# StephenNG59/ICP-symm

Measured on AMD Instinct MI355X. Metric: icp_iterations_per_sec, higher is better.
Workload: dtype f32

## Files before the change

icp-symm_amd/csrc/engine.cpp:

```cpp
#include "engine_internal.h"
#include "robust_loss.h"
#include <limits>

void read_switches(Switches &w)
{
    auto flag = [](const char *n) { return std::getenv(n) != nullptr; };
    auto num = [](const char *n, long def) { const char *e = std::getenv(n); return e ? std::atol(e) : def; };
    auto tri = [](const char *n) { const char *e = std::getenv(n); return e ? (e[0] == '1' ? 1 : 0) : -1; };
    w.allow_any_arch = flag("SYMMICP_ALLOW_ANY_ARCH");
    w.debug_host = flag("SYMMICP_DEBUG_HOST");
    w.debug_counters = flag("SYMMICP_DEBUG_COUNTERS");
    if (const char *e = std::getenv("SYMMICP_DEBUG_TRACE")) w.debug_trace = e;
    if (const char *e = std::getenv("SYMMICP_GRID_PPC")) w.grid_ppc = std::atof(e);
    w.grid_maxlevel = (int)num("SYMMICP_GRID_MAXLEVEL", kMortonBits);
    w.grid_level = (int)num("SYMMICP_GRID_LEVEL", -1);
    if (const char *e = std::getenv("SYMMICP_FIRST_PASS")) w.first_pass = (e[0] == 'p') ? 1 : 0;
    w.oct_leaf = (int)num("SYMMICP_OCT_LEAF", 0);
    if (const char *e = std::getenv("SYMMICP_PACKET_ORDER")) w.packet_order = e[0] != '0';
    if (const char *e = std::getenv("SYMMICP_PACKET_JUMP")) w.packet_jump = (float)std::atof(e);
    w.packet_key_bits = (int)num("SYMMICP_PACKET_KEY_BITS", 16);
    w.packet_chunk = (uint32_t)num("SYMMICP_PACKET_CHUNK", 0);
    w.packet_lds_pad = (uint32_t)num("SYMMICP_PACKET_LDS_PAD", 0);
    w.packet_waves = (uint32_t)num("SYMMICP_PACKET_WAVES", 0);
    w.packet_front_cap = (uint32_t)num("SYMMICP_PACKET_FRONT_CAP", 0);
    if (const char *e = std::getenv("SYMMICP_HOOD_FRAC")) w.hood_frac = std::atof(e);
    w.no_hood = flag("SYMMICP_NO_NEIGHBOURHOOD");
    w.no_cert = flag("SYMMICP_NO_CERT");
    w.walk_full_grid = flag("SYMMICP_WALK_FULL_GRID");
    { const char *e = std::getenv("SYMMICP_HOST_LOOP"); w.host_loop = e && e[0] == '1'; }
    w.no_loop_stragglers = flag("SYMMICP_NO_LOOP_STRAGGLERS");
    w.force_comm = flag("SYMMICP_FORCE_COMM");
    if (const char *e = std::getenv("SYMMICP_PACKET_COST_KEY")) w.packet_cost_key = e[0] != '0';
    w.budget_walk = tri("SYMMICP_BUDGET_WALK");
    w.optimistic = tri("SYMMICP_OPTIMISTIC");
    w.compact = tri("SYMMICP_COMPACT");
    w.pass_blocks = (int)num("SYMMICP_PASS_BLOCKS", 2048);
    w.id_blocks = (int)num("SYMMICP_ID_BLOCKS", 2048);
    w.acc_blocks = (int)num("SYMMICP_ACC_BLOCKS", 512);
    w.fused_blocks = (int)num("SYMMICP_FUSED_BLOCKS", 512);
    w.compact_blocks = (int)num("SYMMICP_COMPACT_BLOCKS", 1280);
    w.feature_nn_splits = (int)num("SYMMICP_FEATURE_NN_SPLITS", 0);
    w.feature_nn_queries = (int)num("SYMMICP_FEATURE_NN_QUERIES", 0);
    w.tune.wave_mode_max = (uint32_t)num("SYMMICP_WAVE_MODE_MAX", 20000);
    w.tune.cells_chunk = (uint32_t)num("SYMMICP_CELLS_CHUNK", 16);
    w.tune.cells_queries = (uint32_t)num("SYMMICP_CELLS_QUERIES", 0);
    w.tune.walk_budget = (uint32_t)num("SYMMICP_WALK_BUDGET", 160);
}

void arena_begin(Arena &a, size_t want)
{
    a.off = 0;
    if (a.cap >= want) return;
    if (a.base) hipFree(a.base);
    a.base = nullptr; a.cap = 0;
    const size_t cap = want + want / 4;
    if (hipMalloc((void **)&a.base, cap) == hipSuccess) a.cap = cap;
    else (void)hipGetLastError();
}


extern "C" {

int symmicp_version(void) { return 100; }

void symmicp_config_default(symmicp_config *cfg)
{
    if (!cfg) return;
    std::memset(cfg, 0, sizeof(*cfg));
    cfg->struct_size = (int32_t)sizeof(*cfg);
    cfg->device = -1;
    cfg->mode = SYMMICP_MODE_QUIRKS;
    cfg->corr = SYMMICP_CORR_IDENTITY;
    cfg->apply = SYMMICP_APPLY_DEFAULT;
    cfg->max_iters = 10;
    cfg->diff_threshold = 1.0f;
    cfg->max_corr_dist = 0.f;
    cfg->fixed_iters = 0;
// ... 1387 lines not shown
```

icp-symm_amd/csrc/engine_debug.cpp:

```cpp
#include "engine_internal.h"

static constexpr size_t kTraceWords = (size_t)1 << 22;
void dump_packet_trace(symmicp_ctx *c)
{
    if (FILE *f = std::fopen(c->sw.debug_trace.c_str(), "wb")) {
        std::vector<unsigned long long> t(kTraceWords);
        hipMemcpy(t.data(), c->dbg_trace, t.size() * 8, hipMemcpyDeviceToHost);
        std::fwrite(t.data(), 8, t.size(), f);
        std::fclose(f);
    }
    hipMemset(c->dbg_trace, 0, kTraceWords * 8);
}


void print_pass_counters(symmicp_ctx *c, bool first, long long list_len)
{
        unsigned long long h[12];
        hipMemcpy(h, c->ix.dbg, sizeof(h), hipMemcpyDeviceToHost);
        hipMemset(c->ix.dbg, 0, sizeof(h));
        if (first && c->cfg.corr == SYMMICP_CORR_TREE && c->target_surface_like)
            std::fprintf(stderr, "[symmicp dbg] pass %lld (packets): steps=%llu nodes+leaf candidates=%llu leaf candidates rejected=%llu points=%llu tie rescans=%llu overflows=%llu lanes wanting a scanned leaf (sum)=%llu | packet ticks (10 ns): sum=%llu max=%llu\n",
                         (long long)c->st.passes, h[0], h[4], h[5], h[3], h[2], h[1], h[8], h[7], h[6]);
        else
        std::fprintf(stderr, "[symmicp dbg] pass %lld: cells: certified=%llu (by neighbourhood %llu) scans=%llu (neighbourhoods kept %llu, not kept %llu) probes=%llu to-walk=%llu items=%llu points=%llu | walk list=%lld visits=%llu wave-max*64=%llu\n",
                     (long long)c->st.passes, h[1], h[8], h[2], h[9], h[10], h[6], h[7], h[0], h[3], list_len, h[4], h[5]);
}
```

icp-symm_amd/csrc/engine_internal.h:

```cpp
#pragma once
#include <hip/hip_runtime.h>
#include <dlfcn.h>
#include <fcntl.h>
#include <sys/mman.h>
#include <sys/stat.h>
#include <unistd.h>
#include <algorithm>
#include <chrono>
#include <cmath>
#include <cstdio>
#include <cstdlib>
#include <cstring>
#include <mutex>
#include <string>
#include <vector>

#include "symmicp.h"
#include "symmicp_internal.h"
#include "host_solve.h"


namespace symmicp {}
using namespace symmicp;

// ... 2 lines not shown
typedef int (*fn_ncclGetUniqueId)(rcclUniqueId *);
typedef int (*fn_ncclCommInitRank)(rcclComm_t *, int, rcclUniqueId, int);
typedef int (*fn_ncclCommDestroy)(rcclComm_t);
typedef int (*fn_ncclAllReduce)(const void *, void *, size_t, int, int, rcclComm_t, hipStream_t);
typedef const char *(*fn_ncclGetErrorString)(int);
constexpr int kNcclFloat64 = 8;
constexpr int kNcclSum = 0;

struct Rccl {
    void *handle = nullptr;
    fn_ncclGetUniqueId GetUniqueId = nullptr;
    fn_ncclCommInitRank CommInitRank = nullptr;
    fn_ncclCommDestroy CommDestroy = nullptr;
    fn_ncclAllReduce AllReduce = nullptr;
    fn_ncclGetErrorString GetErrorString = nullptr;
    std::string err;
    std::mutex mu;
    bool load()
    {
        std::lock_guard<std::mutex> lock(mu);
        if (handle && AllReduce) return true;
        const char *names[] = {"librccl.so.1", "librccl.so"};
        for (const char *nm : names) { handle = dlopen(nm, RTLD_NOW | RTLD_NOLOAD | RTLD_GLOBAL); if (handle) break; }
        if (!handle)
            for (const char *nm : names) { handle = dlopen(nm, RTLD_NOW | RTLD_GLOBAL); if (handle) break; }
        if (!handle) { err = std::string("cannot load librccl: ") + dlerror(); return false; }
        GetUniqueId = (fn_ncclGetUniqueId)dlsym(handle, "ncclGetUniqueId");
        CommInitRank = (fn_ncclCommInitRank)dlsym(handle, "ncclCommInitRank");
        CommDestroy = (fn_ncclCommDestroy)dlsym(handle, "ncclCommDestroy");
        AllReduce = (fn_ncclAllReduce)dlsym(handle, "ncclAllReduce");
        GetErrorString = (fn_ncclGetErrorString)dlsym(handle, "ncclGetErrorString");
        if (!GetUniqueId || !CommInitRank || !CommDestroy || !AllReduce) { err = "librccl misses nccl* symbols"; return false; }
        return true;
    }
};
extern Rccl g_rccl;

inline double now_s()
{
    return std::chrono::duration<double>(std::chrono::steady_clock::now().time_since_epoch()).count();
}

struct Switches {
    bool allow_any_arch = false, debug_host = false, debug_counters = false;
    std::string debug_trace;
    double grid_ppc = 3.0;
    int grid_maxlevel = kMortonBits, grid_level = -1;
    int first_pass = -1;
    int oct_leaf = 0;
    bool packet_order = true;
    bool packet_cost_key = true;
    float packet_jump = -1.0f;
    int packet_key_bits = 16;
    uint32_t packet_chunk = 0, packet_lds_pad = 0, packet_waves = 0, packet_front_cap = 0;
    double hood_frac = 0.8;
    bool no_hood = false, no_cert = false, walk_full_grid = false, host_loop = false, no_loop_stragglers = false, force_comm = false;
    int budget_walk = -1, optimistic = -1, compact = -1;
    int pass_blocks = 2048, id_blocks = 2048, acc_blocks = 512, fused_blocks = 512, compact_blocks = 1280;
    int feature_nn_splits = 0, feature_nn_queries = 0;
    PassTuning tune;
};

void read_switches(Switches &w);

struct Arena {
    char *base = nullptr;
    size_t cap = 0, off = 0;
};

struct ShmSlot {
    volatile unsigned long long seq;
    double s[SYMMICP_NSUM];
    char pad[512 - 8 - 8 * SYMMICP_NSUM];
};
static_assert(sizeof(ShmSlot) == 512, "slot = 4 cache lines");
struct ShmExchange {
    ShmSlot *slots = nullptr;
    size_t bytes = 0;
    unsigned long long count = 0;
    std::string name;
    bool owner = false;
};

struct IndexNotes {
    float origin[3] = {0, 0, 0}, h0 = 0.f;
    uint32_t hist[16] = {};
    uint32_t leaf_max = 0;
    uint32_t nblocks = 0, ctop_len = 0;
};

struct symmicp_ctx {
    Switches sw;
    Arena arena;
    Arena keep;
    std::vector<void *> keep_extra;
    ShmExchange shm;
    symmicp_config cfg{};
    int loss = SYMMICP_LOSS_NONE;
    float loss_scale = 0.f;
    float gicp_eps = 1e-3f;
    float color_lam = 0.968f;
    float4 *tgt_color = nullptr;
    float *src_int = nullptr;
    size_t tgt_color_cap = 0, src_int_cap = 0;
    bool have_tgt_color = false, have_src_int = false;
    float trim_frac = 1.0f;
    uint32_t *trim_keys = nullptr, *trim_ws = nullptr;
// ... 139 lines not shown
```

icp-symm_amd/csrc/engine_loop.cpp:

```cpp
#include "engine_internal.h"

extern "C" {

static void fill_pass_args(symmicp_ctx *c, PassArgs &a, const float Xapply[16], bool from_cur, bool writeback, bool first)
{
    a.in = from_cur ? c->cur : c->src0;
    a.out = c->cur;
    a.n = c->n_loc;
    a.tgt_offset = c->src_off;
    for (int k = 0; k < 12; k++) a.X.m[k] = Xapply[k];
    a.X.nrm_w = (c->cfg.mode == SYMMICP_MODE_QUIRKS) ? 1.0f : 0.0f;
    const bool paper = c->cfg.mode != SYMMICP_MODE_QUIRKS;
    for (int k = 0; k < 3; k++) a.pivot[k] = paper ? c->pivot[k] : 0.0f;
    a.p2p = c->cfg.mode == SYMMICP_MODE_P2P ? 1 : 0;
    a.obj = mode_obj(c->cfg.mode);
    a.gicp_k = 1.0f - c->gicp_eps;
    a.tgt_color = c->tgt_color;
    a.src_int = c->src_int;
    a.color_lam = c->color_lam;
    a.color_om = 1.0f - c->color_lam;
    a.max_d2 = c->cfg.max_corr_dist > 0.f ? c->cfg.max_corr_dist * c->cfg.max_corr_dist : 0.f;
    a.min_ndot = c->cfg.min_normal_dot;
    a.writeback = writeback ? 1 : 0;
    a.best64 = c->best64;
    a.pos_prev = first ? nullptr : c->pos;
    a.pos_out = c->pos;
    a.d2_out = (c->cfg.corr == SYMMICP_CORR_IDENTITY) ? nullptr : c->d2;
    a.partials = c->partials;
    a.cert = reinterpret_cast<float4 *>(c->cert);
    a.certk = c->sw.no_hood ? nullptr : reinterpret_cast<uint4 *>(c->certk);
    a.hoodr = reinterpret_cast<float2 *>(c->hoodr);
    a.make_hood = (a.certk && !first && c->last_uncertified >= 0 && (double)c->last_uncertified < c->sw.hood_frac * (double)c->n_s_total) ? 1 : 0;
    a.pairrec = c->pairrec;
    a.budget_walk = c->sw.budget_walk >= 0 ? c->sw.budget_walk : (first && c->nranks > 1 && c->n_loc < 400000u);
    a.use_slack = (!first && c->cert && !c->sw.no_cert) ? 1 : 0;
    a.loop = nullptr;
    a.pkt_tab = reinterpret_cast<const uint2 *>(c->pkt_tab);
    a.pkt_count = c->pkt_count;
    a.pkt_waves = c->sw.packet_waves;
    a.pkt_front_cap = c->sw.packet_front_cap;
    a.pkt_fallbacks = c->pkt_fallbacks;
    a.pkt_chunk = c->sw.packet_chunk;
    a.pkt_lds_pad = c->sw.packet_lds_pad;
    a.loss = c->loss;
    a.loss_scale = c->loss_scale;
    const bool trim = c->trim_frac < 1.0f && c->trim_keys && c->trim_ws;
    a.trim_keys = trim ? c->trim_keys : nullptr;
    a.trim_ws = trim ? c->trim_ws : nullptr;
    a.trim_host = trim ? reinterpret_cast<uint32_t *>(c->h_sums_dev + kNSum + 1) : nullptr;
    a.trim_rho = c->trim_frac;
}

static int run_pass(symmicp_ctx *c, const float Xapply[16], bool from_cur, bool writeback, bool first)
{
    const bool trim = c->trim_frac < 1.0f;
    if (trim) {
        const size_t want = c->n_loc ? c->n_loc : 1;
        if (c->trim_keys_cap < want) {
            hipFree(c->trim_keys);
            c->trim_keys = nullptr; c->trim_keys_cap = 0;
            HIP_TRY(c, hipMalloc((void **)&c->trim_keys, sizeof(uint32_t) * want));
            c->trim_keys_cap = want;
        }
        if (!c->trim_ws) HIP_TRY(c, hipMalloc((void **)&c->trim_ws, sizeof(uint32_t) * kTrimWsWords));
    }
    c->trim_valid = false;
    PassArgs a{};
    fill_pass_args(c, a, Xapply, from_cur, writeback, first);
    int blocks = (int)((c->n_loc + kPassThreads - 1) / kPassThreads);
    int cap = c->sw.pass_blocks;
    if (cap > 8192) cap = 8192;
    if (blocks > cap) blocks = cap;
    if (blocks < 1) blocks = 1;
    c->pass_blocks = blocks;
    const double t_l0 = now_s();
    if (c->t_last_done > 0) c->t_between += t_l0 - c->t_last_done;
    hipEvent_t *ev = nullptr;
    uint32_t walk_blocks = 0;
    bool optimistic = false;
    if (c->timing) {
        if (c->ev_used == symmicp_ctx::kEvRing) flush_events(c);
        ev = c->ev + c->ev_used * symmicp_ctx::kEvPer;
        c->ev_split[c->ev_used] = (c->timing == 1 || c->timing == 3) ? 1 : 0;
        c->ev_weight[c->ev_used] = 1;
    }
    if (ev && !(c->timing == 2 && c->cfg.corr == SYMMICP_CORR_TREE)) hipEventRecord(ev[0], c->stream);
    switch (c->cfg.corr) {
    case SYMMICP_CORR_IDENTITY: {
        const bool vec4 = (c->n_loc % 4 == 0) && (c->n_t % 4 == 0) && (c->src_off % 4 == 0);
        if (vec4) {
            const int id_cap = c->sw.id_blocks;
            const int nb4 = (int)((c->n_loc / 4 + kPassThreads - 1) / kPassThreads);
            blocks = nb4 < id_cap ? (nb4 > 0 ? nb4 : 1) : id_cap;
// ... 617 lines not shown
```

icp-symm_amd/csrc/kernels_packet.hip:

```cpp
#include <cstdlib>
#include "symmicp_internal.h"
#include "device_common.h"
#pragma clang fp contract(off)

namespace symmicp {

constexpr int kPktStack = 128;
static_assert(kPktStack >= 7 * (kMortonBits + 1) + 1, "packet stack too small for the octree depth");

typedef float f32x16 __attribute__((ext_vector_type(16)));

__device__ __forceinline__ void sload_2x16(const void *p, f32x16 &a, f32x16 &b)
{
    const unsigned long long u = (unsigned long long)p;
    p = (const void *)(((unsigned long long)(uint32_t)__builtin_amdgcn_readfirstlane((int)(u >> 32)) << 32) |
                       (unsigned long long)(uint32_t)__builtin_amdgcn_readfirstlane((int)(uint32_t)u));
    asm volatile("s_load_dwordx16 %0, %2, 0x0\n\ts_load_dwordx16 %1, %2, 0x40\n\ts_waitcnt lgkmcnt(0)" : "=&s"(a), "=&s"(b) : "s"(p) : "memory");
}

template <int CTRL, int ROW_MASK>
__device__ __forceinline__ uint32_t dpp_umax(uint32_t x)
{
    return max(x, (uint32_t)__builtin_amdgcn_update_dpp(0, (int)x, CTRL, ROW_MASK, 0xf, false));
}
// ... 46 lines not shown
{
    const float d2 = dist2(px, py, pz, qx, qy, qz);
    const bool lt = d2 < b.d2;
    tie |= __ballot(d2 == b.d2);
    if (CERT) b.second = min(b.second, max(__float_as_uint(d2), __float_as_uint(b.d2)));
    b.d2 = lt ? d2 : b.d2;
    slot = lt ? K : slot;
}


template <bool CERT>
__device__ __forceinline__ void pkt_leaf_scalar(const float4 *__restrict__ tq, uint32_t first, uint32_t cnt, float px, float py, float pz,
                                                PktBest &b, unsigned long long &c_tie)
{
    for (uint32_t e0 = 0; e0 < cnt; e0 += 8) {
        const uint32_t m = min(cnt - e0, 8u);
        f32x16 qa, qb;
        sload_2x16(tq + first + e0, qa, qb);
        int32_t slot = 8;
        unsigned long long tie = 0;
        pkt_point<CERT, 0>(b, slot, tie, px, py, pz, qa[0], qa[1], qa[2]);
        if (m > 1u) pkt_point<CERT, 1>(b, slot, tie, px, py, pz, qa[4], qa[5], qa[6]);
        if (m > 2u) pkt_point<CERT, 2>(b, slot, tie, px, py, pz, qa[8], qa[9], qa[10]);
        if (m > 3u) pkt_point<CERT, 3>(b, slot, tie, px, py, pz, qa[12], qa[13], qa[14]);
        if (m > 4u) pkt_point<CERT, 4>(b, slot, tie, px, py, pz, qb[0], qb[1], qb[2]);
        if (m > 5u) pkt_point<CERT, 5>(b, slot, tie, px, py, pz, qb[4], qb[5], qb[6]);
        if (m > 6u) pkt_point<CERT, 6>(b, slot, tie, px, py, pz, qb[8], qb[9], qb[10]);
        if (m > 7u) pkt_point<CERT, 7>(b, slot, tie, px, py, pz, qb[12], qb[13], qb[14]);
        if (slot != 8) b.pos = (int32_t)(first + e0) + slot;
        if (tie != 0ull) {
            c_tie++;
            int32_t brow = (b.pos >= 0) ? __float_as_int(tq[b.pos].w) : 0x7fffffff;
#pragma unroll
            for (int k = 0; k < 8; k++) {
                if ((uint32_t)k < m) {
                    const float qx = k < 4 ? qa[4 * k] : qb[4 * (k - 4)], qy = k < 4 ? qa[4 * k + 1] : qb[4 * (k - 4) + 1],
                                qz = k < 4 ? qa[4 * k + 2] : qb[4 * (k - 4) + 2];
                    const int32_t row = __float_as_int(k < 4 ? qa[4 * k + 3] : qb[4 * (k - 4) + 3]);
                    const float d2 = dist2(px, py, pz, qx, qy, qz);
                    if (d2 == b.d2 && row < brow) { brow = row; b.pos = (int32_t)(first + e0) + k; }
                }
            }
        }
    }
}

__device__ __forceinline__ float bcast(float v, int src_lane)
{
    return __int_as_float(__builtin_amdgcn_readlane(__float_as_int(v), src_lane));
}

struct PktCounters {
    unsigned long long nodes, leaves, rejected, points, ties, steps, overflow, wantlanes;
};

template <bool CERT>
__device__ __noinline__ void pkt_dfs(const float4 *__restrict__ onodes, const float4 *__restrict__ tq, const uint32_t *s_off, float4 (*stk)[2],
                                     const float (*s_sb)[8], uint8_t *s_lvl, const int lane, float px, float py, float pz, PktBest &b, float &thr, float pad, PktCounters &cn)
{
    const int sub = lane & 3, chl = lane >> 2;
    const int bperm = (16 * sub + 15) * 4;
    const float4 sblo = *reinterpret_cast<const float4 *>(&s_sb[sub][0]), sbhi = *reinterpret_cast<const float4 *>(&s_sb[sub][4]);
    if (lane == 0) {
        const float4 rA = onodes[0], rB = onodes[1];
        stk[0][0] = rA; stk[0][1] = rB;
        s_lvl[0] = 0;
    }
    int sp = 1;
    __builtin_amdgcn_wave_barrier();
    while (sp > 0) {
        sp--;
        const float4 nA = stk[sp][0], nB = stk[sp][1];
        const bool want = boxdist2(px, py, pz, nA, nB) <= thr;
        if (__ballot(want) == 0ull) { cn.rejected++; continue; }
        const uint32_t first = (uint32_t)__builtin_amdgcn_readfirstlane(__float_as_int(nA.w));
        const uint32_t packed = (uint32_t)__builtin_amdgcn_readfirstlane(__float_as_int(nB.w));
        const uint32_t level = s_lvl[sp], nch = oct_nch(packed), cf = oct_cf(packed);
        if (nch == 0) {
            cn.leaves++; cn.points += cf;
            pkt_leaf_scalar<CERT>(tq, first, cf, px, py, pz, b, cn.ties);
            thr = fminf(thr, pkt_threshold(b.d2, pad));
        } else {
            cn.nodes++;
            const uint32_t tb = (thr >= 0.0f) ? __float_as_uint(thr) + 1u : 0u;
            const uint32_t thr_g = (uint32_t)__builtin_amdgcn_ds_bpermute(bperm, (int)row_umax(tb));
            uint32_t bbd = 0x7f800000u;
            float4 cA = make_float4(0.f, 0.f, 0.f, 0.f), cB = cA;
            const bool mine = (lane < 32) && ((uint32_t)chl < nch);
            if (mine) {
                const float4 *__restrict__ ch = onodes + 2 * ((size_t)s_off[level + 1] + cf + (uint32_t)chl);
                cA = ch[0]; cB = ch[1];
                const float gx = fmaxf(fmaxf(cA.x - sbhi.x, sblo.x - cB.x), 0.0f);
                const float gy = fmaxf(fmaxf(cA.y - sbhi.y, sblo.y - cB.y), 0.0f);
                const float gz = fmaxf(fmaxf(cA.z - sbhi.z, sblo.z - cB.z), 0.0f);
                bbd = __float_as_uint((gx * gx + gy * gy) + gz * gz);
            }
            const bool keep = mine && bbd < thr_g;
            const uint32_t m32 = (uint32_t)__ballot(keep);
            if (m32) {
                uint32_t mc = m32 | (m32 >> 1);
                mc = (mc | (mc >> 2)) & 0x11111111u;
                uint32_t key = keep ? ((bbd & ~7u) | (uint32_t)chl) : 0xFFFFFFFFu;
                key = dpp_umin<0xB1, 0xf>(key);
                key = dpp_umin<0x4E, 0xf>(key);
                key = dpp_umin<0x114, 0xf>(key);
                key = dpp_umin<0x118, 0xf>(key);
                const uint32_t kmin = min((uint32_t)__builtin_amdgcn_readlane((int)key, 15), (uint32_t)__builtin_amdgcn_readlane((int)key, 31));
                const uint32_t cmin = kmin & 7u;
                const uint32_t nk = (uint32_t)__popc(mc);
                const uint32_t rank = (uint32_t)__popc(mc & ((1u << (4 * (chl & 7))) - 1u));
                const uint32_t rmin = (uint32_t)__popc(mc & ((1u << (4 * cmin)) - 1u));
                if (mine && sub == 0 && ((mc >> (4 * (chl & 7))) & 1u)) {
                    const uint32_t slot = ((uint32_t)chl == cmin) ? nk - 1u : (rank > rmin ? rank - 1u : rank);
                    stk[sp + slot][0] = cA; stk[sp + slot][1] = cB;
                    s_lvl[sp + slot] = (uint8_t)(level + 1u);
                }
                sp += (int)nk;
            }
            __builtin_amdgcn_wave_barrier();
        }
    }
}

template <int ND, bool DBG>
__device__ __forceinline__ bool pkt_step(const uint32_t *fr_cur, uint32_t *fr_next, uint32_t nf, uint32_t f0, uint32_t off_next, uint32_t *cnt_next, uint32_t front_cap, int lane,
                                         const float4 *__restrict__ onodes, const float4 *__restrict__ tq, float px, float py, float pz, bool wants,
                                         const float (&gl)[4][3], const float (&gh)[4][3], const uint32_t (&dive)[ND], PktBest &b, float &thr, PktCounters &cn)
{
    constexpr bool CERT = false;
    const float pad = 0.0f;
    uint32_t tg[4];
    {
        const uint32_t tb = wants ? __float_as_uint(thr) + 1u : 0u;
        const uint32_t r = row_umax(tb);
#pragma unroll
        for (int g = 0; g < 4; g++) tg[g] = (uint32_t)__builtin_amdgcn_readlane((int)r, 16 * g + 15);
    }
    const uint32_t f = f0 + (uint32_t)(lane >> 3), c = (uint32_t)(lane & 7);
    const uint32_t pkd = (f < nf) ? fr_cur[f] : 0u;
    const bool valid = c < oct_nch(pkd);
    float4 cA = make_float4(0.f, 0.f, 0.f, 0.f), cB = cA;
    bool keep = false;
    if (valid) {
        const float4 *__restrict__ ch = onodes + 2 * ((size_t)off_next + oct_cf(pkd) + c);
        cA = ch[0]; cB = ch[1];
#pragma unroll
        for (int g = 0; g < 4; g++) {
            const float gx = fmaxf(fmaxf(cA.x - gh[g][0], gl[g][0] - cB.x), 0.0f);
            const float gy = fmaxf(fmaxf(cA.y - gh[g][1], gl[g][1] - cB.y), 0.0f);
            const float gz = fmaxf(fmaxf(cA.z - gh[g][2], gl[g][2] - cB.z), 0.0f);
            keep |= __float_as_uint((gx * gx + gy * gy) + gz * gz) < tg[g];
        }
    }
    const uint32_t cpk = (uint32_t)__float_as_int(cB.w);
    const bool isleaf = oct_nch(cpk) == 0u;
    const bool keepL = keep && isleaf, keepI = keep && !isleaf;
    if (DBG) cn.nodes += (unsigned long long)__popcll(__ballot(valid));
    const unsigned long long mI = __ballot(keepI);
    if (mI) {
        uint32_t base = 0;
        if (lane == 0) base = atomicAdd(cnt_next, (uint32_t)__popcll(mI));
        base = (uint32_t)__builtin_amdgcn_readfirstlane((int)base);
        const uint32_t dst = base + __builtin_amdgcn_mbcnt_hi((uint32_t)(mI >> 32), __builtin_amdgcn_mbcnt_lo((uint32_t)mI, 0u));
        if (keepI && dst < front_cap) fr_next[dst] = cpk;
    }
    unsigned long long mL = __ballot(keepL);
    bool scanned = false;
    if (mL) {
        while (mL) {
            const int src = (int)__ffsll((long long)mL) - 1;
            mL &= mL - 1ull;
            if (DBG) cn.leaves++;
            const uint32_t lfirst = (uint32_t)__builtin_amdgcn_readlane(__float_as_int(cA.w), src);
            bool dived = false;
#pragma unroll
            for (int w = 0; w < ND; w++) dived |= (lfirst == dive[w]);
            if (dived) continue;
            float4 lo, hi;
            lo.x = bcast(cA.x, src); lo.y = bcast(cA.y, src); lo.z = bcast(cA.z, src);
            hi.x = bcast(cB.x, src); hi.y = bcast(cB.y, src); hi.z = bcast(cB.z, src);
            const unsigned long long mw = __ballot(boxdist2(px, py, pz, lo, hi) <= thr);
            if (mw == 0ull) { if (DBG) cn.rejected++; continue; }
            if (DBG) cn.wantlanes += (unsigned long long)__popcll(mw);
            const uint32_t cnt = oct_cf((uint32_t)__builtin_amdgcn_readlane((int)cpk, src));
            if (DBG) cn.points += cnt;
            pkt_leaf_scalar<CERT>(tq, lfirst, cnt, px, py, pz, b, cn.ties);
            thr = fminf(thr, pkt_threshold(b.d2, pad));
            scanned = true;
        }
    }
    return scanned;
}

constexpr int kFrontCap = 512;
static_assert(2 * kFrontCap * sizeof(uint32_t) <= kPktStack * 2 * sizeof(float4), "frontier buffers alias the DFS stack");
constexpr int kPktLevels = kMortonBits + 3;

template <int W>
__device__ __forceinline__ void pkt_sync()
{
    if (W == 1) __builtin_amdgcn_wave_barrier();
    else __syncthreads();
}

#ifndef PKT_WAVES1
#define PKT_WAVES1 5
#endif
#ifndef PKT_WAVESN
#define PKT_WAVESN 5
#endif
template <int W, bool DBG>
__global__ __launch_bounds__(64 * W, W == 1 ? PKT_WAVES1 : PKT_WAVESN) void k_search_packet(PassArgs a, TargetIndex ix, uint32_t chunk)
{
    __shared__ float4 s_buf[kPktStack][2];
    __shared__ float s_sb[4][8];
    __shared__ uint8_t s_lvl[kPktStack];
    __shared__ uint32_t s_off[kMortonBits + 2];
    __shared__ uint32_t s_cnt[kPktLevels];
    __shared__ uint32_t s_stp[kPktLevels];
    __shared__ uint32_t s_thr[64];
    __shared__ unsigned long long s_key[64];
    __shared__ uint32_t s_dive[W];
    uint32_t (*fr)[kFrontCap] = reinterpret_cast<uint32_t (*)[kFrontCap]>(&s_buf[0][0]);
    const int lane = threadIdx.x & 63;
    const int wave = (W == 1) ? 0 : __builtin_amdgcn_readfirstlane((int)(threadIdx.x >> 6));
    const float inf = __int_as_float(0x7f800000);
    if (threadIdx.x < kMortonBits + 2) s_off[threadIdx.x] = ix.olevel_off[threadIdx.x];
    __syncthreads();
    const uint32_t npk = a.pkt_tab ? a.pkt_count : (a.n + 63u) >> 6;
    const uint32_t front_cap = min(a.pkt_front_cap ? a.pkt_front_cap : (uint32_t)kFrontCap, (uint32_t)kFrontCap);
    constexpr bool CERT = false;
    const float pad = 0.0f;
    const float4 *__restrict__ tq = ix.tq;
    const float4 *__restrict__ onodes = ix.onodes;
    PktCounters cn = {0, 0, 0, 0, 0, 0, 0, 0};
    for (uint32_t slot = xcd_remap_chunked(blockIdx.x, chunk); slot < npk; slot += gridDim.x) {
        uint32_t first = slot * 64u, count = 64u;
        if (a.pkt_tab) { const uint2 e = a.pkt_tab[slot]; first = e.x; count = e.y; }
        const uint32_t pk = slot;
        unsigned long long t_start = 0;
        if (DBG || ix.dbg_trace) t_start = __builtin_amdgcn_s_memrealtime();
        const PktCounters cn0 = cn;
        if (wave == 0) {
            if (lane < kPktLevels) { s_cnt[lane] = 0; s_stp[lane] = 0; }
            if (W > 1) { s_thr[lane] = 0x7f800000u; s_key[lane] = ~0ull; }
            if (lane < W) s_dive[lane] = 0xFFFFFFFFu;
        }
        pkt_sync<W>();
        const uint32_t i = first + (uint32_t)lane;
        const bool active = (uint32_t)lane < count && i < a.n;
        float px = 0.f, py = 0.f, pz = 0.f;
        PktBest b;
        b.d2 = inf; b.second = 0x7f800000u; b.pos = -1;
        float thr = -1.0f;
        if (active) {
            const float x = a.in.x[i], y = a.in.y[i], z = a.in.z[i];
            px = xf_row(a.X.m + 0, x, y, z, 1.0f); py = xf_row(a.X.m + 4, x, y, z, 1.0f); pz = xf_row(a.X.m + 8, x, y, z, 1.0f);
            thr = ((px == px) & (py == py) & (pz == pz)) ? inf : -1.0f;
        }
        const bool wants = thr >= 0.0f;
        const unsigned long long wants0 = __ballot(wants);
        uint32_t steps_pk = 0;
        bool ovf_pk = false;
        if (wants0 != 0ull) {
            float gl[4][3], gh[4][3];
            {
                const float lx = row_fmin(wants ? px : inf), ly = row_fmin(wants ? py : inf), lz = row_fmin(wants ? pz : inf);
                const float hx = row_fmax(wants ? px : -inf), hy = row_fmax(wants ? py : -inf), hz = row_fmax(wants ? pz : -inf);
#pragma unroll
                for (int g = 0; g < 4; g++) {
                    gl[g][0] = bcast(lx, 16 * g + 15); gl[g][1] = bcast(ly, 16 * g + 15); gl[g][2] = bcast(lz, 16 * g + 15);
                    gh[g][0] = bcast(hx, 16 * g + 15); gh[g][1] = bcast(hy, 16 * g + 15); gh[g][2] = bcast(hz, 16 * g + 15);
                }
                if (wave == 0 && (lane & 15) == 15) {
                    float *sb = const_cast<float *>(s_sb[lane >> 4]);
                    sb[0] = lx; sb[1] = ly; sb[2] = lz; sb[3] = 0.f; sb[4] = hx; sb[5] = hy; sb[6] = hz; sb[7] = 0.f;
                }
            }
            const float4 rootA = onodes[0], rootB = onodes[1];
            const uint32_t root_first = (uint32_t)__builtin_amdgcn_readfirstlane(__float_as_int(rootA.w));
            const uint32_t root_packed = (uint32_t)__builtin_amdgcn_readfirstlane(__float_as_int(rootB.w));
            bool done = false;
            {
                const int nw = __popcll(wants0);
                int kth = ((2 * wave + 1) * nw) / (2 * W);
                unsigned long long m = wants0;
                while (kth-- > 0) m &= m - 1ull;
                const int mid = (int)__ffsll((long long)m) - 1;
                const float cx = bcast(px, mid), cy = bcast(py, mid), cz = bcast(pz, mid);
                uint32_t packed = root_packed, dfirst = root_first, level = 0;
                while (oct_nch(packed) != 0u) {
                    const uint32_t nch = oct_nch(packed), cf = oct_cf(packed);
                    uint32_t key = 0xFFFFFFFFu;
                    float4 cA = make_float4(0.f, 0.f, 0.f, 0.f), cB = cA;
                    if ((uint32_t)lane < nch) {
                        const float4 *__restrict__ ch = onodes + 2 * ((size_t)s_off[level + 1] + cf + (uint32_t)lane);
                        cA = ch[0]; cB = ch[1];
                        key = (__float_as_uint(boxdist2(cx, cy, cz, cA, cB)) & ~7u) | (uint32_t)lane;
                    }
                    key = dpp_umin<0x111, 0xf>(key); key = dpp_umin<0x112, 0xf>(key); key = dpp_umin<0x114, 0xf>(key);
                    const int cmin = __builtin_amdgcn_readlane((int)key, 7) & 7;
                    packed = (uint32_t)__builtin_amdgcn_readlane(__float_as_int(cB.w), cmin);
                    dfirst = (uint32_t)__builtin_amdgcn_readlane(__float_as_int(cA.w), cmin);
                    level++;
                    if (DBG) cn.steps++;
                }
                const uint32_t cnt = oct_cf(packed);
                if (DBG) cn.points += cnt;
                pkt_leaf_scalar<CERT>(tq, dfirst, cnt, px, py, pz, b, cn.ties);
                thr = fminf(thr, pkt_threshold(b.d2, pad));
                done = (level == 0);
                if (lane == 0) s_dive[wave] = dfirst;
                if (W > 1 && wants) atomicMin(&s_thr[lane], __float_as_uint(thr));
            }
            if (!done && wave == 0 && lane == 0) { fr[0][0] = root_packed; s_cnt[0] = 1u; }
            pkt_sync<W>();
            uint32_t dive_w[W];
#pragma unroll
            for (int w = 0; w < W; w++) dive_w[w] = s_dive[w];
            int cur = 0;
            bool overflow = false;
            for (uint32_t level = 0; !done; level++) {
                const uint32_t nf = s_cnt[level];
                if (nf == 0u) break;
                if (nf > front_cap) { overflow = true; break; }
                const uint32_t off_next = s_off[level + 1];
                uint32_t my_step = 0;
                while (true) {
                    uint32_t st = my_step++;
                    if (W > 1) {
                        if (lane == 0) st = atomicAdd(&s_stp[level], 1u);
                        st = (uint32_t)__builtin_amdgcn_readfirstlane((int)st);
                    }
                    const uint32_t f0 = st * 8u;
                    if (f0 >= nf) break;
                    if (DBG) { cn.steps++; steps_pk++; }
                    if (W > 1 && wants) thr = __uint_as_float(min(__float_as_uint(thr), s_thr[lane]));
                    const bool scanned = pkt_step<W, DBG>(fr[cur], fr[cur ^ 1], nf, f0, off_next, &s_cnt[level + 1], front_cap, lane, onodes, tq, px, py, pz, wants, gl, gh, dive_w, b, thr, cn);
                    if (W > 1 && scanned && wants) thr = __uint_as_float(min(__float_as_uint(thr), atomicMin(&s_thr[lane], __float_as_uint(thr))));
                }
                cur ^= 1;
                pkt_sync<W>();
            }
            if (overflow) {
                ovf_pk = true;
                if (wave == 0) {
                    cn.overflow++;
                    if (lane == 0 && a.pkt_fallbacks) atomicAdd(a.pkt_fallbacks, 1u);
                    if (W > 1 && wants) thr = __uint_as_float(min(__float_as_uint(thr), s_thr[lane]));
                    PktBest b2 = b;
                    float thr2 = thr;
                    PktCounters cn2 = {0, 0, 0, 0, 0, 0, 0, 0};
                    pkt_dfs<CERT>(onodes, tq, s_off, s_buf, s_sb, s_lvl, lane, px, py, pz, b2, thr2, pad, cn2);
                    b = b2; thr = thr2;
                    if (DBG) { cn.nodes += cn2.nodes; cn.leaves += cn2.leaves; cn.rejected += cn2.rejected; cn.points += cn2.points; cn.ties += cn2.ties; }
                }
            }
        }
        bool writer = (wave == 0);
        if (W > 1) {
            unsigned long long key = ~0ull;
            if (active && b.pos >= 0) key = ((unsigned long long)__float_as_uint(b.d2) << 32) | (unsigned long long)(uint32_t)__float_as_int(tq[b.pos].w);
            if (key != ~0ull) atomicMin(&s_key[lane], key);
            __syncthreads();
            const unsigned long long kmin = s_key[lane];
            writer = (kmin == ~0ull) ? (wave == 0) : (key == kmin);
            if (kmin == ~0ull) b.pos = -1;
        }
        if (active && writer) {
            a.pos_out[i] = b.pos;
            a.d2_out[i] = b.d2;
            a.cert[i] = make_float4(px, py, pz, 0.0f);
            if (b.pos >= 0) store_pair_record(a, ix, i, b.pos);
            else a.pairrec[2 * (size_t)i + 1] = make_float4(0.f, 0.f, 0.f, 1.f);
        }
        if (!DBG && ix.dbg_trace && wave == 0 && lane == 0 && (size_t)pk < ((size_t)1 << 21)) {
            const unsigned long long dt = __builtin_amdgcn_s_memrealtime() - t_start;
            ix.dbg_trace[2 * (size_t)pk] = t_start;
            ix.dbg_trace[2 * (size_t)pk + 1] = (dt << 32) | (unsigned long long)((first << 1) | (ovf_pk ? 1u : 0u));
        }
        if (DBG && lane == 0) {
            const unsigned long long dt = __builtin_amdgcn_s_memrealtime() - t_start;
            if (wave == 0) { atomicMax(ix.dbg + 6, dt); atomicAdd(ix.dbg + 7, dt); }
            if (ix.dbg_trace && (size_t)pk < ((size_t)1 << 18)) {
                unsigned long long *tr = ix.dbg_trace + 8 * (size_t)pk;
                if (wave == 0) { tr[0] = t_start; tr[1] = (dt << 32) | (unsigned long long)((first << 1) | (ovf_pk ? 1u : 0u)); }
                tr[2 + wave] = ((unsigned long long)(steps_pk & 0xFFFFu) << 48) | ((unsigned long long)((cn.leaves - cn.rejected - cn0.leaves + cn0.rejected) & 0xFFFFu) << 32) |
                               ((unsigned long long)((cn.points - cn0.points) & 0xFFFFFFu) << 8) | (unsigned long long)((cn.ties - cn0.ties) & 0xFFu);
                if (wave == 0) tr[6] = ((unsigned long long)(cn.nodes - cn0.nodes) << 32) | (unsigned long long)(cn.leaves - cn0.leaves);
            }
        }
        if (W > 1) __syncthreads();
    }
    if (DBG && lane == 0) {
        atomicAdd(ix.dbg + 0, cn.steps);
        atomicAdd(ix.dbg + 1, cn.overflow);
        atomicAdd(ix.dbg + 2, cn.ties);
        atomicAdd(ix.dbg + 3, cn.points);
        atomicAdd(ix.dbg + 4, cn.nodes + cn.leaves);
        atomicAdd(ix.dbg + 5, cn.rejected);
        atomicAdd(ix.dbg + 8, cn.wantlanes);
    }
}

constexpr float kJumpFactor = 4.5f;
constexpr float kMedianSteps = 6.0f;
constexpr int kMaxRunsPerBlock = 8;

__global__ __launch_bounds__(64) void k_packet_runs(CloudSoA src, uint32_t n, float jump_factor, uint2 *__restrict__ runs, uint32_t *__restrict__ keys,
                                                    uint32_t *__restrict__ vals, uint32_t *__restrict__ count, int key_bits)
{
    const uint32_t i = blockIdx.x * 64u + threadIdx.x;
    const int lane = threadIdx.x;
    const bool active = i < n;
    const float x = active ? src.x[i] : 0.f, y = active ? src.y[i] : 0.f, z = active ? src.z[i] : 0.f;
    float sx = x, sy = y, sz = z, cnt = active ? 1.f : 0.f;
#pragma unroll
    for (int off = 1; off < 16; off <<= 1) {
        sx += __shfl_xor(sx, off, 64); sy += __shfl_xor(sy, off, 64); sz += __shfl_xor(sz, off, 64); cnt += __shfl_xor(cnt, off, 64);
    }
    float r16 = active ? dist2(x, y, z, sx / cnt, sy / cnt, sz / cnt) : 0.f;
#pragma unroll
    for (int off = 1; off < 16; off <<= 1) r16 = fmaxf(r16, __shfl_xor(r16, off, 64));
    float scale2 = (cnt >= 8.f) ? r16 : __int_as_float(0x7f800000);
    scale2 = fminf(scale2, __shfl_xor(scale2, 16, 64));
    scale2 = fminf(scale2, __shfl_xor(scale2, 32, 64));
    const float px = __shfl_up(x, 1, 64), py = __shfl_up(y, 1, 64), pz = __shfl_up(z, 1, 64);
    const bool has_step = active && lane > 0;
    const float step2 = has_step ? dist2(x, y, z, px, py, pz) : __int_as_float(0x7f800000);
    const int nsteps = __popcll(__ballot(has_step));
    int rank = 0;
    for (int j = 1; j < 64; j++) {
        const float o = __shfl(step2, j, 64);
        rank += (o < step2 || (o == step2 && j < lane)) ? 1 : 0;
    }
    {
        const unsigned long long mm = __ballot(has_step && rank == (nsteps - 1) / 2);
        if (nsteps >= 3 && mm) {
            const float med2 = __shfl(step2, (int)__ffsll((long long)mm) - 1, 64);
            scale2 = fminf(scale2, kMedianSteps * kMedianSteps * med2);
        }
    }
    const bool jump = has_step && jump_factor > 0.f && step2 > jump_factor * jump_factor * scale2 && rank >= nsteps - (kMaxRunsPerBlock - 1);
    const unsigned long long cuts = __ballot(jump) | 1ull;
    const unsigned long long act = __ballot(active);
    const unsigned long long below = cuts & ((2ull << lane) - 1ull);
    const int start = 63 - __clzll((long long)below);
    const unsigned long long above = cuts & ~((2ull << lane) - 1ull);
    const int nact = __popcll(act);
    const int end = above ? (int)__ffsll((long long)above) - 1 : nact;
    float cx = 0.f, cy = 0.f, cz = 0.f, r2 = 0.f;
    for (unsigned long long m = cuts; m; m &= m - 1) {
        const int s0 = (int)__ffsll((long long)m) - 1;
        const bool mine = active && start == s0;
// ... 123 lines not shown
```

icp-symm_amd/csrc/symmicp_internal.h:

```cpp
#pragma once
#include <hip/hip_runtime.h>
#include <stdint.h>
#include <stddef.h>
#include "symmicp.h"

namespace symmicp {

constexpr int kNSum = SYMMICP_NSUM;
constexpr int kNAcc = 37;
constexpr int kNAccW = 38;
constexpr double kListDropped = 4294967296.0;
constexpr int kLeaf = 8;
constexpr int kFan = 8;
constexpr int kMaxTreeLevels = 12;
constexpr int kMortonBits = 10;
constexpr int kPassThreads = 256;
constexpr int kBruteTile = 1024;
constexpr int kBruteQ = 4;

constexpr bool mode_device_solves(int mode)
{
    return mode == SYMMICP_MODE_QUIRKS || mode == SYMMICP_MODE_PAPER || mode == SYMMICP_MODE_PLANE || mode == SYMMICP_MODE_GICP;
}
constexpr bool mode_known(int mode) { return mode_device_solves(mode) || mode == SYMMICP_MODE_P2P || mode == SYMMICP_MODE_COLOR; }
// ... 56 lines not shown
    int32_t stop;
    int32_t reason;
    int32_t iters;
    int32_t small_step;
};
enum { LOOP_RUNNING = 0, LOOP_DONE = 1, LOOP_REDO_PASS = 2, LOOP_HOST_SOLVE = 3, LOOP_SLOW = 4 };
struct LoopConfig {
    int32_t mode, fixed_iters, max_iters, incremental, tree;
    float diff_threshold, eps_rotation, eps_translation, nrm_w;
    float pivot[3];
    uint32_t uncertified_limit;
    int32_t walk_in_loop;
    uint32_t list_limit;
};
struct LoopRecord {
    double sums[SYMMICP_NSUM];
    float increment[16], X[16];
    float rcond;
    int32_t status;
    int32_t solved;
    int32_t pad;
    int32_t list_len, reserved;
};

struct PassArgs {
    CloudSoA in, out;
    uint32_t n;
    uint32_t tgt_offset;
    Affine X;
    float pivot[3];
    float max_d2;
    float min_ndot;
    int32_t p2p;
    int32_t writeback;
    const unsigned long long *best64;
    int32_t *pos_prev;
    float *d2_out;
    int32_t *pos_out;
    double *partials;
    float4 *pairrec;
    int32_t budget_walk;
    int32_t refresh_records;
    float4 *cert;
    uint4 *certk;
    float2 *hoodr;
    int32_t make_hood;
    int32_t use_slack;
    const LoopState *loop;
    uint32_t partial_cols, partial_col0;
    const uint2 *pkt_tab;
    uint32_t pkt_count;
    uint32_t pkt_waves;
    uint32_t pkt_front_cap;
    uint32_t *pkt_fallbacks;
    uint32_t pkt_chunk, pkt_lds_pad;
    int32_t loss;
    float loss_scale;
    int32_t obj;
    float gicp_k;
    uint32_t *trim_keys;
    uint32_t *trim_ws;
    uint32_t *trim_host;
    float trim_rho;
    const float4 *tgt_color;
    const float *src_int;
    float color_lam, color_om;
};
constexpr uint32_t kTrimWsWords = 16 + 3 * 2048;
constexpr uint32_t kTrimTauWord = 3;

struct PassTuning {
    uint32_t wave_mode_max = 20000u;
    uint32_t cells_chunk = 16u;
    uint32_t cells_queries = 0u;
    uint32_t walk_budget = 160u;
};

void launch_pass_identity(const PassArgs &a, CloudSoA tgt, int blocks, bool vec4_ok, hipStream_t s);
void launch_pass_indexed(const PassArgs &a, const float4 *tn , int blocks, hipStream_t s);
void launch_pass_tree_split(const PassArgs &a, const TargetIndex &ix, const WorkLists &wl, int acc_blocks, uint32_t walk_blocks,
                            int stage, int compact_blocks, const PassTuning &tune, hipStream_t s, hipEvent_t *ev);
void launch_pass_tree_first(const PassArgs &a, const TargetIndex &ix, const WorkLists &wl, int acc_blocks, hipStream_t s, hipEvent_t *ev);
uint32_t walk_blocks_full(const WorkLists &wl);
uint32_t shard_capacity(uint32_t n_points);
void launch_final_reduce(const double *partials, int blocks, double *out_dev, double *out_host_mapped, uint32_t *ticket,
                         unsigned long long seq, uint32_t *counters_to_clear, int keep_nonempty, hipStream_t s);
void launch_pass_fused(const PassArgs &a, const TargetIndex &ix, const WorkLists &wl, int blocks, hipStream_t s);
void launch_loop_stragglers(const PassArgs &a, const TargetIndex &ix, const WorkLists &wl, int list_blocks, const PassTuning &tune, hipStream_t s);
void launch_reduce_solve(const double *partials, int blocks, double *out_dev, int mode, LoopState *loop, LoopConfig cfg, LoopRecord *ring, int ring_len,
                         uint32_t *counters_to_clear, hipStream_t s);
void launch_solve_probe(int mode, int exact_rc, const symmicp_sums *sums, int n, const float *pivot, const float *X_in, int32_t *status, float *pbar,
                        float *qbar, float *a, float *t, float *rcond, float *out16, float *X_out, hipStream_t s);
void launch_loop_end(const LoopState *loop, LoopState *host_copy, unsigned long long *done_flag, unsigned long long seq, hipStream_t s);
void launch_publish(const double *sums_dev, double *out_host_mapped, unsigned long long seq, hipStream_t s);
void launch_nn_brute(const CloudSoA &src, uint32_t n_s, const Affine &X, const float4 *tq, uint32_t n_t,
                     unsigned long long *best64, hipStream_t s);

void launch_bbox(const float *x, const float *y, const float *z, uint32_t n, uint32_t *bbox_ord6, hipStream_t s);
void launch_morton(const float *x, const float *y, const float *z, uint32_t n, float ox, float oy, float oz,
                   float inv_h0, uint32_t *keys, uint32_t *vals, hipStream_t s);
void radix_sort_pairs(uint32_t *keys, uint32_t *vals, uint32_t *keys_tmp, uint32_t *vals_tmp, uint32_t n,
                      int key_bits, uint32_t *hist_ws, size_t hist_ws_elems, hipStream_t s);
size_t radix_sort_ws_elems(uint32_t n);
void launch_gather_f4(const float *x, const float *y, const float *z, const float *nx, const float *ny, const float *nz,
                      const uint32_t *order, uint32_t n, float4 *tq, float4 *tn, hipStream_t s);
void launch_gather_soa(const CloudSoA &src, const uint32_t *order, uint32_t n, CloudSoA dst, hipStream_t s);
// ... 63 lines not shown
```

Before: 30300.

## Batch packet leaf scans into per-wave item queue drained lane-parallel

Replaces the per-leaf scalar scan in the packet traversal step with a per-wave LDS work queue. Each query lane that wants a leaf pushes chunks of 8 points as items, and these are drained in parallel, one item per lane, with atomicMin merging into per-query keys. The goal is to cut the serial broadcast scans when only a few lanes want each leaf. In exchange it adds LDS footprint (items, keys, positions per wave), extra barriers and drain overhead, and new debug counters.

```diff
diff --git a/icp-symm_amd/csrc/engine.cpp b/icp-symm_amd/csrc/engine.cpp
--- a/icp-symm_amd/csrc/engine.cpp
+++ b/icp-symm_amd/csrc/engine.cpp
@@ -23,6 +23,7 @@
     w.packet_lds_pad = (uint32_t)num("SYMMICP_PACKET_LDS_PAD", 0);
     w.packet_waves = (uint32_t)num("SYMMICP_PACKET_WAVES", 0);
     w.packet_front_cap = (uint32_t)num("SYMMICP_PACKET_FRONT_CAP", 0);
+    w.packet_item_cap = (uint32_t)num("SYMMICP_PACKET_ITEM_CAP", 0);
     if (const char *e = std::getenv("SYMMICP_HOOD_FRAC")) w.hood_frac = std::atof(e);
     w.no_hood = flag("SYMMICP_NO_NEIGHBOURHOOD");
     w.no_cert = flag("SYMMICP_NO_CERT");
diff --git a/icp-symm_amd/csrc/engine_debug.cpp b/icp-symm_amd/csrc/engine_debug.cpp
--- a/icp-symm_amd/csrc/engine_debug.cpp
+++ b/icp-symm_amd/csrc/engine_debug.cpp
@@ -19,8 +19,8 @@
         hipMemcpy(h, c->ix.dbg, sizeof(h), hipMemcpyDeviceToHost);
         hipMemset(c->ix.dbg, 0, sizeof(h));
         if (first && c->cfg.corr == SYMMICP_CORR_TREE && c->target_surface_like)
-            std::fprintf(stderr, "[symmicp dbg] pass %lld (packets): steps=%llu nodes+leaf candidates=%llu leaf candidates rejected=%llu points=%llu tie rescans=%llu overflows=%llu lanes wanting a scanned leaf (sum)=%llu | packet ticks (10 ns): sum=%llu max=%llu\n",
-                         (long long)c->st.passes, h[0], h[4], h[5], h[3], h[2], h[1], h[8], h[7], h[6]);
+            std::fprintf(stderr, "[symmicp dbg] pass %lld (packets): steps=%llu nodes+leaf candidates=%llu leaf candidates rejected=%llu points=%llu tie rescans=%llu overflows=%llu lanes wanting a scanned leaf (sum)=%llu items pushed=%llu drain rounds=%llu lane-tests executed=%llu | packet ticks (10 ns): sum=%llu max=%llu\n",
+                         (long long)c->st.passes, h[0], h[4], h[5], h[3], h[2], h[1], h[8], h[9], h[10], h[11], h[7], h[6]);
         else
         std::fprintf(stderr, "[symmicp dbg] pass %lld: cells: certified=%llu (by neighbourhood %llu) scans=%llu (neighbourhoods kept %llu, not kept %llu) probes=%llu to-walk=%llu items=%llu points=%llu | walk list=%lld visits=%llu wave-max*64=%llu\n",
                      (long long)c->st.passes, h[1], h[8], h[2], h[9], h[10], h[6], h[7], h[0], h[3], list_len, h[4], h[5]);
diff --git a/icp-symm_amd/csrc/engine_internal.h b/icp-symm_amd/csrc/engine_internal.h
--- a/icp-symm_amd/csrc/engine_internal.h
+++ b/icp-symm_amd/csrc/engine_internal.h
@@ -78,7 +78,7 @@
     bool packet_cost_key = true;
     float packet_jump = -1.0f;
     int packet_key_bits = 16;
-    uint32_t packet_chunk = 0, packet_lds_pad = 0, packet_waves = 0, packet_front_cap = 0;
+    uint32_t packet_chunk = 0, packet_lds_pad = 0, packet_waves = 0, packet_front_cap = 0, packet_item_cap = 0;
     double hood_frac = 0.8;
     bool no_hood = false, no_cert = false, walk_full_grid = false, host_loop = false, no_loop_stragglers = false, force_comm = false;
     int budget_walk = -1, optimistic = -1, compact = -1;
diff --git a/icp-symm_amd/csrc/engine_loop.cpp b/icp-symm_amd/csrc/engine_loop.cpp
--- a/icp-symm_amd/csrc/engine_loop.cpp
+++ b/icp-symm_amd/csrc/engine_loop.cpp
@@ -39,6 +39,7 @@
     a.pkt_count = c->pkt_count;
     a.pkt_waves = c->sw.packet_waves;
     a.pkt_front_cap = c->sw.packet_front_cap;
+    a.pkt_item_cap = c->sw.packet_item_cap;
     a.pkt_fallbacks = c->pkt_fallbacks;
     a.pkt_chunk = c->sw.packet_chunk;
     a.pkt_lds_pad = c->sw.packet_lds_pad;
diff --git a/icp-symm_amd/csrc/kernels_packet.hip b/icp-symm_amd/csrc/kernels_packet.hip
--- a/icp-symm_amd/csrc/kernels_packet.hip
+++ b/icp-symm_amd/csrc/kernels_packet.hip
@@ -122,6 +122,9 @@
 
 struct PktCounters {
     unsigned long long nodes, leaves, rejected, points, ties, steps, overflow, wantlanes;
+};
+struct PktItemCounters {
+    unsigned long long items, rounds, lanetests;
 };
 
 template <bool CERT>
@@ -192,13 +195,73 @@
     }
 }
 
+constexpr int kItemCap = 320;
+constexpr int kItemChunk = 8;
+#ifndef PKT_WIDE_LANES
+#define PKT_WIDE_LANES 65
+#endif
+#ifndef PKT_DRAIN_MARK
+#define PKT_DRAIN_MARK 192
+#endif
+
+template <bool DBG>
+__device__ __forceinline__ void pkt_drain(const uint2 *items, uint32_t n, unsigned long long *wkey, int32_t *wpos, int lane, const float4 *__restrict__ tq,
+                                          float px, float py, float pz, PktBest &b, float &thr, PktItemCounters &ic)
+{
+    __builtin_amdgcn_wave_barrier();
+    for (uint32_t r0 = 0; r0 < n; r0 += 64u) {
+        const uint32_t it = r0 + (uint32_t)lane;
+        uint2 item = make_uint2(0u, 0u);
+        if (it < n) item = items[it];
+        const int q = (int)(item.y & 63u);
+        const uint32_t cnt = item.y >> 8;
+        const float qx = __int_as_float(__builtin_amdgcn_ds_bpermute(4 * q, __float_as_int(px)));
+        const float qy = __int_as_float(__builtin_amdgcn_ds_bpermute(4 * q, __float_as_int(py)));
+        const float qz = __int_as_float(__builtin_amdgcn_ds_bpermute(4 * q, __float_as_int(pz)));
+        const float4 *__restrict__ pt = tq + item.x;
+        unsigned long long key = ~0ull;
+        int32_t kbest = -1;
+#pragma unroll
+        for (int h = 0; h < kItemChunk; h += 4) {
+            float4 t[4];
+#pragma unroll
+            for (int k = 0; k < 4; k++) t[k] = pt[h + k];
+#pragma unroll
+            for (int k = 0; k < 4; k++) {
+                const float d2 = dist2(qx, qy, qz, t[k].x, t[k].y, t[k].z);
+                const unsigned long long kk = ((unsigned long long)__float_as_uint(d2) << 32) | (unsigned long long)(uint32_t)__float_as_int(t[k].w);
+                const bool lt = ((uint32_t)(h + k) < cnt) & (kk < key);
+                key = lt ? kk : key;
+                kbest = lt ? h + k : kbest;
+            }
+        }
+        const int32_t pos = (kbest >= 0 && (uint32_t)(key >> 32) <= 0x7f800000u) ? (int32_t)item.x + kbest : -1;
+        if (pos >= 0) atomicMin(&wkey[q], key);
+        __builtin_amdgcn_wave_barrier();
+        if (pos >= 0 && wkey[q] == key) wpos[q] = pos;
+        __builtin_amdgcn_wave_barrier();
+        if (DBG) { ic.rounds++; ic.lanetests += (unsigned long long)kItemChunk; }
+    }
+    const unsigned long long k = wkey[lane];
+    if (k != ~0ull) {
+        const float kd2 = __uint_as_float((uint32_t)(k >> 32));
+        const int32_t kpos = wpos[lane];
+        bool take = kd2 < b.d2;
+        if (kd2 == b.d2 && kpos != b.pos) {
+            const int32_t brow = (b.pos >= 0) ? __float_as_int(tq[b.pos].w) : 0x7fffffff;
+            take = (int32_t)(uint32_t)k < brow;
+        }
+        if (take) { b.d2 = kd2; b.pos = kpos; }
+    }
+    thr = fminf(thr, pkt_threshold(b.d2, 0.0f));
+}
+
 template <int ND, bool DBG>
 __device__ __forceinline__ bool pkt_step(const uint32_t *fr_cur, uint32_t *fr_next, uint32_t nf, uint32_t f0, uint32_t off_next, uint32_t *cnt_next, uint32_t front_cap, int lane,
                                          const float4 *__restrict__ onodes, const float4 *__restrict__ tq, float px, float py, float pz, bool wants,
-                                         const float (&gl)[4][3], const float (&gh)[4][3], const uint32_t (&dive)[ND], PktBest &b, float &thr, PktCounters &cn)
-{
-    constexpr bool CERT = false;
-    const float pad = 0.0f;
+                                         const float (&gl)[4][3], const float (&gh)[4][3], const uint32_t (&dive)[ND], uint2 *items, uint32_t &nit, uint32_t item_cap,
+                                         unsigned long long *wkey, int32_t *wpos, PktBest &b, float &thr, PktCounters &cn, PktItemCounters &ic)
+{
     uint32_t tg[4];
     {
         const uint32_t tb = wants ? __float_as_uint(thr) + 1u : 0u;
@@ -235,31 +298,45 @@
         if (keepI && dst < front_cap) fr_next[dst] = cpk;
     }
     unsigned long long mL = __ballot(keepL);
-    bool scanned = false;
-    if (mL) {
-        while (mL) {
-            const int src = (int)__ffsll((long long)mL) - 1;
-            mL &= mL - 1ull;
-            if (DBG) cn.leaves++;
-            const uint32_t lfirst = (uint32_t)__builtin_amdgcn_readlane(__float_as_int(cA.w), src);
-            bool dived = false;
-#pragma unroll
-            for (int w = 0; w < ND; w++) dived |= (lfirst == dive[w]);
-            if (dived) continue;
-            float4 lo, hi;
-            lo.x = bcast(cA.x, src); lo.y = bcast(cA.y, src); lo.z = bcast(cA.z, src);
-            hi.x = bcast(cB.x, src); hi.y = bcast(cB.y, src); hi.z = bcast(cB.z, src);
-            const unsigned long long mw = __ballot(boxdist2(px, py, pz, lo, hi) <= thr);
-            if (mw == 0ull) { if (DBG) cn.rejected++; continue; }
-            if (DBG) cn.wantlanes += (unsigned long long)__popcll(mw);
-            const uint32_t cnt = oct_cf((uint32_t)__builtin_amdgcn_readlane((int)cpk, src));
-            if (DBG) cn.points += cnt;
-            pkt_leaf_scalar<CERT>(tq, lfirst, cnt, px, py, pz, b, cn.ties);
-            thr = fminf(thr, pkt_threshold(b.d2, pad));
-            scanned = true;
-        }
-    }
-    return scanned;
+    bool improved = false;
+    while (mL) {
+        const int src = (int)__ffsll((long long)mL) - 1;
+        mL &= mL - 1ull;
+        if (DBG) cn.leaves++;
+        const uint32_t lfirst = (uint32_t)__builtin_amdgcn_readlane(__float_as_int(cA.w), src);
+        bool dived = false;
+#pragma unroll
+        for (int w = 0; w < ND; w++) dived |= (lfirst == dive[w]);
+        if (dived) continue;
+        float4 lo, hi;
+        lo.x = bcast(cA.x, src); lo.y = bcast(cA.y, src); lo.z = bcast(cA.z, src);
+        hi.x = bcast(cB.x, src); hi.y = bcast(cB.y, src); hi.z = bcast(cB.z, src);
+        const bool mine = boxdist2(px, py, pz, lo, hi) <= thr;
+        const unsigned long long mw = __ballot(mine);
+        if (mw == 0ull) { if (DBG) cn.rejected++; continue; }
+        const uint32_t nw = (uint32_t)__popcll(mw);
+        if (DBG) cn.wantlanes += (unsigned long long)nw;
+        const uint32_t cnt = oct_cf((uint32_t)__builtin_amdgcn_readlane((int)cpk, src));
+        if (DBG) cn.points += cnt;
+        if (PKT_WIDE_LANES <= 64 && nw >= (uint32_t)PKT_WIDE_LANES) {
+            if (DBG) ic.lanetests += cnt;
+            pkt_leaf_scalar<false>(tq, lfirst, cnt, px, py, pz, b, cn.ties);
+            thr = fminf(thr, pkt_threshold(b.d2, 0.0f));
+            improved = true;
+            continue;
+        }
+        const uint32_t rank = __builtin_amdgcn_mbcnt_hi((uint32_t)(mw >> 32), __builtin_amdgcn_mbcnt_lo((uint32_t)mw, 0u));
+        for (uint32_t e0 = 0; e0 < cnt; e0 += (uint32_t)kItemChunk) {
+            if (nit + nw > item_cap) {
+                pkt_drain<DBG>(items, nit, wkey, wpos, lane, tq, px, py, pz, b, thr, ic);
+                nit = 0; improved = true;
+            }
+            if (mine) items[nit + rank] = make_uint2(lfirst + e0, (uint32_t)lane | (min(cnt - e0, (uint32_t)kItemChunk) << 8));
+            nit += nw;
+            if (DBG) ic.items += (unsigned long long)nw;
+        }
+    }
+    return improved;
 }
 
 constexpr int kFrontCap = 512;
@@ -291,6 +368,9 @@
     __shared__ uint32_t s_thr[64];
     __shared__ unsigned long long s_key[64];
     __shared__ uint32_t s_dive[W];
+    __shared__ uint2 s_item[W][kItemCap];
+    __shared__ unsigned long long s_wkey[W][64];
+    __shared__ int32_t s_wpos[W][64];
     uint32_t (*fr)[kFrontCap] = reinterpret_cast<uint32_t (*)[kFrontCap]>(&s_buf[0][0]);
     const int lane = threadIdx.x & 63;
     const int wave = (W == 1) ? 0 : __builtin_amdgcn_readfirstlane((int)(threadIdx.x >> 6));
@@ -299,11 +379,13 @@
     __syncthreads();
     const uint32_t npk = a.pkt_tab ? a.pkt_count : (a.n + 63u) >> 6;
     const uint32_t front_cap = min(a.pkt_front_cap ? a.pkt_front_cap : (uint32_t)kFrontCap, (uint32_t)kFrontCap);
+    const uint32_t item_cap = max(min(a.pkt_item_cap ? a.pkt_item_cap : (uint32_t)kItemCap, (uint32_t)kItemCap), 64u);
     constexpr bool CERT = false;
     const float pad = 0.0f;
     const float4 *__restrict__ tq = ix.tq;
     const float4 *__restrict__ onodes = ix.onodes;
     PktCounters cn = {0, 0, 0, 0, 0, 0, 0, 0};
+    PktItemCounters ic = {0, 0, 0};
     for (uint32_t slot = xcd_remap_chunked(blockIdx.x, chunk); slot < npk; slot += gridDim.x) {
         uint32_t first = slot * 64u, count = 64u;
         if (a.pkt_tab) { const uint2 e = a.pkt_tab[slot]; first = e.x; count = e.y; }
@@ -316,6 +398,7 @@
             if (W > 1) { s_thr[lane] = 0x7f800000u; s_key[lane] = ~0ull; }
             if (lane < W) s_dive[lane] = 0xFFFFFFFFu;
         }
+        s_wkey[wave][lane] = ~0ull;
         pkt_sync<W>();
         const uint32_t i = first + (uint32_t)lane;
         const bool active = (uint32_t)lane < count && i < a.n;
@@ -376,7 +459,7 @@
                     if (DBG) cn.steps++;
                 }
                 const uint32_t cnt = oct_cf(packed);
-                if (DBG) cn.points += cnt;
+                if (DBG) { cn.points += cnt; ic.lanetests += cnt; }
                 pkt_leaf_scalar<CERT>(tq, dfirst, cnt, px, py, pz, b, cn.ties);
                 thr = fminf(thr, pkt_threshold(b.d2, pad));
                 done = (level == 0);
@@ -390,6 +473,7 @@
             for (int w = 0; w < W; w++) dive_w[w] = s_dive[w];
             int cur = 0;
             bool overflow = false;
+            uint32_t nit = 0;
             for (uint32_t level = 0; !done; level++) {
                 const uint32_t nf = s_cnt[level];
                 if (nf == 0u) break;
@@ -403,11 +487,20 @@
                         st = (uint32_t)__builtin_amdgcn_readfirstlane((int)st);
                     }
                     const uint32_t f0 = st * 8u;
-                    if (f0 >= nf) break;
-                    if (DBG) { cn.steps++; steps_pk++; }
-                    if (W > 1 && wants) thr = __uint_as_float(min(__float_as_uint(thr), s_thr[lane]));
-                    const bool scanned = pkt_step<W, DBG>(fr[cur], fr[cur ^ 1], nf, f0, off_next, &s_cnt[level + 1], front_cap, lane, onodes, tq, px, py, pz, wants, gl, gh, dive_w, b, thr, cn);
-                    if (W > 1 && scanned && wants) thr = __uint_as_float(min(__float_as_uint(thr), atomicMin(&s_thr[lane], __float_as_uint(thr))));
+                    const bool last = f0 >= nf;
+                    bool improved = false;
+                    if (!last) {
+                        if (DBG) { cn.steps++; steps_pk++; }
+                        if (W > 1 && wants) thr = __uint_as_float(min(__float_as_uint(thr), s_thr[lane]));
+                        improved = pkt_step<W, DBG>(fr[cur], fr[cur ^ 1], nf, f0, off_next, &s_cnt[level + 1], front_cap, lane, onodes, tq, px, py, pz, wants, gl, gh, dive_w,
+                                                    s_item[wave], nit, item_cap, s_wkey[wave], s_wpos[wave], b, thr, cn, ic);
+                    }
+                    if (nit != 0u && (last || nit >= (uint32_t)PKT_DRAIN_MARK)) {
+                        pkt_drain<DBG>(s_item[wave], nit, s_wkey[wave], s_wpos[wave], lane, tq, px, py, pz, b, thr, ic);
+                        nit = 0; improved = true;
+                    }
+                    if (W > 1 && improved && wants) thr = __uint_as_float(min(__float_as_uint(thr), atomicMin(&s_thr[lane], __float_as_uint(thr))));
+                    if (last) break;
                 }
                 cur ^= 1;
                 pkt_sync<W>();
@@ -423,7 +516,7 @@
                     PktCounters cn2 = {0, 0, 0, 0, 0, 0, 0, 0};
                     pkt_dfs<CERT>(onodes, tq, s_off, s_buf, s_sb, s_lvl, lane, px, py, pz, b2, thr2, pad, cn2);
                     b = b2; thr = thr2;
-                    if (DBG) { cn.nodes += cn2.nodes; cn.leaves += cn2.leaves; cn.rejected += cn2.rejected; cn.points += cn2.points; cn.ties += cn2.ties; }
+                    if (DBG) { cn.nodes += cn2.nodes; cn.leaves += cn2.leaves; cn.rejected += cn2.rejected; cn.points += cn2.points; cn.ties += cn2.ties; ic.lanetests += cn2.points; }
                 }
             }
         }
@@ -470,6 +563,9 @@
         atomicAdd(ix.dbg + 4, cn.nodes + cn.leaves);
         atomicAdd(ix.dbg + 5, cn.rejected);
         atomicAdd(ix.dbg + 8, cn.wantlanes);
+        atomicAdd(ix.dbg + 9, ic.items);
+        atomicAdd(ix.dbg + 10, ic.rounds);
+        atomicAdd(ix.dbg + 11, ic.lanetests * 64ull);
     }
 }
 
diff --git a/icp-symm_amd/csrc/symmicp_internal.h b/icp-symm_amd/csrc/symmicp_internal.h
--- a/icp-symm_amd/csrc/symmicp_internal.h
+++ b/icp-symm_amd/csrc/symmicp_internal.h
@@ -132,6 +132,7 @@
     uint32_t pkt_count;
     uint32_t pkt_waves;
     uint32_t pkt_front_cap;
+    uint32_t pkt_item_cap;
     uint32_t *pkt_fallbacks;
     uint32_t pkt_chunk, pkt_lds_pad;
     int32_t loss;
```

After: 30350 (median of 2 runs). No clear change (+0.2%).
